# osmosis-diffusion/osmosis-diffusion-code

Measured on AMD Instinct MI355X. Metric: denoise-steps/sec (256x256 RGBD, 1000-step DDPM+guidance), higher is better.
Workload: dtype f32 (f16x3 conv)

## Files before the change

### osmosis_diffusion_code_amd/_lib.py

```python
import ctypes as C
import os
import threading
from typing import List, Optional, Tuple

import torch

_HERE = os.path.dirname(os.path.abspath(__file__))
LIB_PATH = os.environ.get("OSM_LIB") or os.path.join(_HERE, "libosmosis_hip.so")

c_float_p = C.c_void_p


class OsmosisHipError(RuntimeError):
    pass


class ConvDesc(C.Structure):
    _fields_ = [("x", C.c_void_p), ("w", C.c_void_p), ("bias", C.c_void_p), ("res", C.c_void_p),
                ("y", C.c_void_p), ("splitk_ws", C.c_void_p),
                ("B", C.c_int), ("H", C.c_int), ("W", C.c_int), ("Cin", C.c_int), ("Cout", C.c_int),
                ("ksize", C.c_int), ("splitk", C.c_int), ("accumulate", C.c_int),
                ("ldx", C.c_longlong), ("ldy", C.c_longlong), ("ldr", C.c_longlong), ("wfmt", C.c_int),
                ("gn_table", C.c_void_p), ("gn_silu", C.c_int),
                ("colsum", C.c_void_p), ("stat_mode", C.c_int), ("stat_silu", C.c_int), ("stat_x", C.c_void_p),
# ... 153 lines not shown
    "osm_version": [],
}
for _n in ("osm_conv2d_nhwc", "osm_gn_stats", "osm_gn_apply", "osm_gn_fwd", "osm_gn_prep", "osm_gn_bwd", "osm_gn_bwd_apply", "osm_pool2x2",
           "osm_resample_pair", "osm_upsample2x", "osm_stride2_pick", "osm_stride2_place", "osm_add_rowvec", "osm_nchw_to_nhwc", "osm_nhwc_to_nchw", "osm_copy2d"):
    _SIGS[_n + "_h"] = _SIGS[_n]
_SIGS["osm_half_to_f32"] = [_P, _LL, _P, _LL, _LL, _I, _P]
_SIGS["osm_f32_to_half"] = [_P, _LL, _P, _LL, _LL, _I, _P]
EXPORTS = sorted(list(_SIGS) + ["osm_last_error", "osm_packed_weight_elems", "osm_winograd_weight_elems", "osm_quantile_abs_ws_bytes"])
_SIGS_LINOP = {
    "osm_linop_apply": [_P, _P, _P, _P, _P, _P, _I, _I, _LL, _LL, _I, _I, _I, _I, _I, _I, _I, _P],
}
EXPORTS_LINOP = sorted(_SIGS_LINOP)
_SIGS_PSF = {
    "osm_psf_apply": [_P, _P, _P, _P, _P, _I, _I, _I, _I, _I, _LL, _LL, _I, _I, _I, _I, _P],
}
EXPORTS_PSF = sorted(_SIGS_PSF)
_SIGS_PHYSLIN = {
    "osm_phys_forward": [C.POINTER(PhysDesc), _P, _P, _P, _P],
    "osm_phys_resid": [C.POINTER(PhysDesc), _I, _P, _P, _P, _P, _P, _P],
    "osm_phys_reduce_lin": [C.POINTER(PhysDesc), _P, _P, _P, _P, _P],
    "osm_phys_finalize_lin": [C.POINTER(PhysDesc), _I, _P, _P, _P, _P, _I, _P, _P, _I, _P],
    "osm_phys_grad_lin": [C.POINTER(PhysDesc), _I, _P, _P, _P, _P, _P, _I, _P],
    "osm_phys_optimize_lin": [C.POINTER(PhysDesc), C.POINTER(LinDesc), _P, _P, _P, _P, _P, _P, _P, _P, _P, _P, _P, _P, _P, _I, _I, _P, _P],
}
EXPORTS_PHYSLIN = sorted(_SIGS_PHYSLIN)
_SIGS_PHYSGROUP = {
    "osm_phys_finalize_g": [C.POINTER(PhysDesc), C.POINTER(GroupDesc), _P, _P, _P, _I, _P, _P, _I, _P],
    "osm_phys_finalize_lin_g": [C.POINTER(PhysDesc), C.POINTER(GroupDesc), _I, _P, _P, _P, _P, _I, _P, _P, _I, _P],
    "osm_phys_optimize_g": [C.POINTER(PhysDesc), C.POINTER(GroupDesc), _P, _P, _P, _P, _P, _P, _P, _P, _I, _I, _P, _P],
    "osm_phys_optimize_lin_g": [C.POINTER(PhysDesc), C.POINTER(GroupDesc), C.POINTER(LinDesc), _P, _P, _P, _P, _P, _P, _P, _P, _P, _P, _P,
                                _P, _P, _I, _I, _P, _P],
}
EXPORTS_PHYSGROUP = sorted(_SIGS_PHYSGROUP)
_D = C.c_double
_SIGS_BLIND = {
    "osm_psf_tap_grad": [_P, _P, _P, _P, _I, _I, _I, _I, _I, _LL, _LL, _I, _I, _P, _P],
    "osm_psf_tap_step": [_P, _P, _P, _I, _I, _I, _LL, _D, _D, _P],
    "osm_ps_blind_optimize": [_P, _P, _P, _P, _P, _P, _I, _I, _I, _I, _I, _I, _I, _P, _P, _P, _P, _P, _P, _I, _D, _D, _P],
}
EXPORTS_BLIND = sorted(_SIGS_BLIND)
_SIGS_DEPTHPRIOR = {
    "osm_depth_nblk": [_I],
    "osm_depth_reduce": [C.POINTER(DepthDesc), _P, _P, _P, _P, _P],
    "osm_depth_fit": [C.POINTER(DepthDesc), _P, _P, _P, _P],
    "osm_depth_grad": [C.POINTER(DepthDesc), _P, _P, _P, _P, _P, _P],
    "osm_depth_loss_grad": [C.POINTER(DepthDesc), _P, _P, _P, _P, _P, _P, _P, _P],
}
EXPORTS_DEPTHPRIOR = sorted(_SIGS_DEPTHPRIOR)
_SIGS_SOLVER = {
    "osm_solver_update_c": [_P, _P, _P, _P, _P, _P, _P, _P, _P, _F, _P, _P, _P, _I, _I, _I, _P],
    "osm_solver_update_rng_c": [_P, _P, _P, _P, _P, _P, _P, _P, _F, _P, _P, _P, _I, _I, _I, C.c_ulonglong, _P, _I, _I, _I, _I, _P],
}
EXPORTS_SOLVER = sorted(_SIGS_SOLVER)

_lib = None
_lock = threading.Lock()


def load():
    global _lib
    if _lib is not None:
        return _lib
    with _lock:
        if _lib is None:
            if not os.path.exists(LIB_PATH):
                raise OsmosisHipError(
                    f"{LIB_PATH} is missing: build it with `python -c 'import __graft_entry__ as g; g.build()'` "
                    "or `make -C osmosis_diffusion_code_amd/csrc` (hipcc, --offload-arch=gfx950). "
                    "There is no CPU fallback for the product path.")
            lib = C.CDLL(LIB_PATH)
            for name, argtypes in list(_SIGS.items()) + list(_SIGS_LINOP.items()) + list(_SIGS_PSF.items()) + list(_SIGS_PHYSLIN.items()) + \
                    list(_SIGS_PHYSGROUP.items()) + list(_SIGS_BLIND.items()) + list(_SIGS_DEPTHPRIOR.items()) + list(_SIGS_SOLVER.items()):
                fn = getattr(lib, name)
                fn.argtypes = argtypes
                fn.restype = C.c_int
            lib.osm_packed_weight_elems.argtypes = [_I, _I, _I, _I, _I]
            lib.osm_packed_weight_elems.restype = C.c_longlong
            lib.osm_winograd_weight_elems.argtypes = [_I, _I, _I, _I]
            lib.osm_winograd_weight_elems.restype = C.c_longlong
            lib.osm_quantile_abs_ws_bytes.argtypes = [_LL]
            lib.osm_quantile_abs_ws_bytes.restype = C.c_longlong
            lib.osm_last_error.argtypes = []
            lib.osm_last_error.restype = C.c_char_p
            _lib = lib
    return _lib


class Recorder:

    def __init__(self):
        self.calls: List[Tuple] = []
        self.keep: List = []

    def __enter__(self):
        _state.recorders.append(self)
        return self

    def __exit__(self, *exc):
        _state.recorders.pop()
        return False

    @staticmethod
    def suspended():
        class _Suspend:
            def __enter__(self_):
                self_.saved, _state.recorders = _state.recorders, []

            def __exit__(self_, *exc):
                _state.recorders = self_.saved
                return False
        return _Suspend()

    def replay(self):
        for c in self.calls:
            fn, args = c[0], c[1]
            rc = fn(*args)
            if rc != 0:
                raise OsmosisHipError(f"{fn.__name__} failed ({rc}): {load().osm_last_error().decode()}")

    def to_graph(self):
        g = torch.cuda.CUDAGraph()
        cap = torch.cuda.Stream()
        cap.wait_stream(torch.cuda.current_stream())
        with torch.cuda.graph(g, stream=cap):
            cs = torch.cuda.current_stream()
# ... 78 lines not shown
```

### osmosis_diffusion_code_amd/csrc/guidance.hip

```cpp
#include "osm_common.h"
#include "depth_conv.h"
#include "../../include/osmosis_linop.h"
#include "../../include/osmosis_psf.h"
#include "../../include/osmosis_physlin.h"
#include "../../include/osmosis_physgroup.h"
#include "../../include/osmosis_solver.h"

namespace {

constexpr int PPB = 1024;
constexpr int NRED = 16;

template <bool MASKED> struct PixMask { float wm[3]; };
template <> struct PixMask<false> {};

template <bool MASKED>
struct Pix : PixMask<MASKED> {
  float rgb[3], D, y[3];
  float d, dd, w;
  float Ea[3], Eb[3], J[3], r[3];
};

template <bool MASKED, bool FMA_I = false, bool MODEL_ONLY = false>
__device__ __forceinline__ void eval_pixel(const osm_phys_desc& ds, const float* __restrict__ x0,
                                           const float* __restrict__ y, const float* __restrict__ mask,
                                           const float* __restrict__ phi, int b, int p, Pix<MASKED>& q) {
  const long long base = (long long)b * 4 * ds.HW + p;
  float m[3] = {1.f, 1.f, 1.f};
#pragma unroll
  for (int c = 0; c < 3; ++c) {
    q.rgb[c] = x0[base + (long long)c * ds.HW];
    if constexpr (!MODEL_ONLY) q.y[c] = y[(long long)b * 3 * ds.HW + (long long)c * ds.HW + p];
    if constexpr (MASKED) m[c] = mask[(long long)b * 3 * ds.HW + (long long)c * ds.HW + p];
  }
  q.D = x0[base + 3LL * ds.HW];
  if (ds.kind == 3) {
    q.d = 0.f; q.dd = 0.f; q.w = 1.f;
#pragma unroll
    for (int c = 0; c < 3; ++c) {
      q.Ea[c] = q.Eb[c] = 1.f;
      q.J[c] = 0.5f * (q.rgb[c] + 1.0f);
      q.r[c] = q.y[c] - q.rgb[c];
      if constexpr (MASKED) { q.wm[c] = m[c]; q.r[c] *= m[c]; }
    }
    return;
  }
  q.d = conv_depth(q.D, ds.depth_type, ds.dval, q.dd);
  float wdd;
  q.w = ds.weight_type == 1 ? conv_depth(q.D, ds.wdepth_type, ds.wval, wdd) : 1.0f;
  const float* ph = phi + b * 9;
#pragma unroll
  for (int c = 0; c < 3; ++c) {
    const float pa = ds.kind == 2 ? ph[0] : ph[c];
    const float pb = ds.kind == 0 ? ph[3 + c] : pa;
    const float pinf = ph[6 + c];
    q.Ea[c] = expf(-pa * q.d);
    q.Eb[c] = expf(-pb * q.d);
    q.J[c] = 0.5f * (q.rgb[c] + 1.0f);
    float I;
// ... 134 lines not shown
      ph[i] += -lr[i] * (g[i] / (sqrtf(sq) + (float)1e-8));
    }
  } else if (ds.optimizer == 5) {
    for (int i = 0; i < 9; ++i) {
      if (!((live >> i) & 1) || lr[i] == 0.f) continue;
      const float sm = st[i] + g[i] * g[i];
      st[i] = sm;
      ph[i] += -lr[i] * (g[i] / (sqrtf(sm) + (float)1e-10));
    }
  } else if (ds.optimizer == 6) {
    for (int i = 0; i < 9; ++i) {
      if (!((live >> i) & 1) || lr[i] == 0.f) continue;
      const float sq = st[i] * (float)0.9 + (float)(1.0 - 0.9) * g[i] * g[i];
      const float sd = sqrtf(sq + (float)1e-6);
      const float dl = sqrtf(st[9 + i] + (float)1e-6) / sd * g[i];
      st[i] = sq;
      st[9 + i] = st[9 + i] * (float)0.9 + (float)(1.0 - 0.9) * dl * dl;
      ph[i] += -lr[i] * dl;
    }
  } else if (ds.optimizer == 7) {
    const float step = st[19] + 1.f;
    st[19] = step;
    for (int i = 0; i < 9; ++i) {
      if (!((live >> i) & 1) || lr[i] == 0.f) continue;
      const float eta = step == 1.f ? lr[i] : st[i];
      ph[i] *= (float)(1.0 - 1e-4 * (double)eta);
      ph[i] += -eta * g[i];
      st[i] = (float)((double)lr[i] / pow(1.0 + 1e-4 * (double)lr[i] * (double)step, 0.75));
    }
  } else if (ds.optimizer == 8) {
    const float step = st[18] + 1.f;
    st[18] = step;
    for (int i = 0; i < 9; ++i) {
      if (!((live >> i) & 1) || lr[i] == 0.f) continue;
      float ss = step == 1.f ? lr[i] : st[9 + i];
      const float pr = g[i] * st[i];
      float gi = g[i];
      ss *= pr > 0.f ? 1.2f : (pr < 0.f ? 0.5f : 1.f);
      ss = fminf(fmaxf(ss, 1e-6f), 50.f);
      if (pr < 0.f) gi = 0.f;
      ph[i] += -(sgn(gi) * ss);
      st[i] = gi; st[9 + i] = ss;
    }
  } else {
    for (int i = 0; i < 9; ++i)
      if ((live >> i) & 1) ph[i] -= lr[i] * g[i];
  }
  if (ds.kind == 2) ph[1] = ph[2] = ph[0];
}

template <bool LIN> struct FinLin { const float* part_r; int nblk_r, hw; };
template <> struct FinLin<false> {};

template <bool LIN>
__device__ __forceinline__ void fin_walk(const float* __restrict__ part, float* __restrict__ red, int nblk, const FinLin<LIN>& lin,
                                         int b, int lane, double* tot) {
  static_assert(NRED * 4 == 64, "one wave covers the components");
  const int comp = lane >> 2, sub = lane & 3;
  double a = 0.0;
#pragma unroll 4
  for (int k = sub; k < nblk; k += 4) a += (double)part[((long long)b * nblk + k) * NRED + comp];
  if constexpr (LIN) {
    if (comp == 0) {
      a = 0.0;
      for (int k = sub; k < lin.nblk_r; k += 4) a += (double)lin.part_r[(long long)b * lin.nblk_r + k];
    }
  }
  a += __shfl_xor(a, 1, 64);
  a += __shfl_xor(a, 2, 64);
  if (sub == 0) {
    tot[comp] = a;
    red[b * NRED + comp] = (float)a;
  }
}

template <bool LIN>
__device__ __forceinline__ bool fin_member(const osm_phys_desc& ds, const double* tot, const FinLin<LIN>& lin, int zero_guard, int b,
                                           float* __restrict__ loss_out, int do_update, double* dg) {
  double n = 3.0 * (double)ds.HW;
  if constexpr (LIN) n = 3.0 * (double)lin.hw;
  double L, gscale;
  bool live = true;
  if (ds.loss_type == 0) {
    L = sqrt(tot[0]);
    gscale = 1.0 / L;
    if (zero_guard && tot[0] == 0.0) { gscale = 0.0; live = false; }
  } else {
    L = tot[0] / n;
    gscale = 2.0 / n;
  }
  if (loss_out) loss_out[b] = (float)L;
  if (do_update) phys_param_grad(ds, tot, gscale, dg);
  return live;
}

__device__ __forceinline__ void fin_step(const osm_phys_desc& ds, const double* dg, double omega, float* ph, float* st) {
  float g[9], lr[9];
  const int live = phys_param_lr(ds, lr);
  for (int i = 0; i < 9; ++i) g[i] = (float)(dg[i] * omega);
  phys_opt_step(ds, g, lr, live, ph, st);
}

template <bool LIN>
__global__ void phys_finalize_kernel(osm_phys_desc ds, const float* __restrict__ part, float* __restrict__ red,
                                     float* __restrict__ phi, int do_update, float* __restrict__ loss_out,
                                     float* __restrict__ opt_state, int nblk, int zero_guard, const FinLin<LIN> lin) {
  __shared__ double tot[NRED];
  const int b = blockIdx.x;
  fin_walk(part, red, nblk, lin, b, threadIdx.x, tot);
  __syncthreads();
  if (threadIdx.x == 0) {
    double dg[9];
    if (fin_member(ds, tot, lin, zero_guard, b, loss_out, do_update, dg) && do_update)
      fin_step(ds, dg, 1.0, phi + b * 9, opt_state ? opt_state + b * 20 : nullptr);
// ... 56 lines not shown
__global__ __launch_bounds__(256) void phys_grad_kernel(osm_phys_desc ds, const float* __restrict__ x0,
                                                         const float* __restrict__ y,
                                                         const float* __restrict__ mask,
                                                         const float* __restrict__ phi, const float* __restrict__ v,
                                                         const float* __restrict__ red, float* __restrict__ g, int hw,
                                                         int zero_guard) {
  static_assert(!(MASKED && LIN), "the composed route's mask acts on the measurement's grid (phys_resid_kernel)");
  const int b = blockIdx.y;
  const int p = blockIdx.x * 256 + threadIdx.x;
  if (p >= ds.HW) return;
  Pix<MASKED> q;
  eval_pixel<MASKED, MASKED, LIN>(ds, x0, y, mask, phi, b, p, q);
  const float* rd = red + b * NRED;
  const float n = 3.0f * (float)ds.HW;
  float gscale = ds.loss_type == 0 ? 1.0f / sqrtf(rd[0]) : 2.0f / (LIN ? 3.0f * (float)hw : n);
  if ((MASKED || (LIN && zero_guard)) && ds.loss_type == 0 && rd[0] == 0.f) gscale = 0.f;
  const float* ph = phi + b * 9;
  float gD = 0.f;
  const long long base = (long long)b * 4 * ds.HW + p;
  if constexpr (!LIN) {
    if (ds.kind == 3) {
#pragma unroll
      for (int c = 0; c < 3; ++c) {
        if constexpr (MASKED) g[base + (long long)c * ds.HW] = -(q.wm[c] * (q.r[c] * gscale));
        else g[base + (long long)c * ds.HW] = -(q.r[c] * gscale);
      }
      g[base + 3LL * ds.HW] = 0.f;
      return;
    }
  }
#pragma unroll
  for (int c = 0; c < 3; ++c) {
    const float pa = ds.kind == 2 ? ph[0] : ph[c];
    const float pb = ds.kind == 0 ? ph[3 + c] : pa;
    const float pinf = ph[6 + c];
    float dLdI;
    if constexpr (LIN) {
      dLdI = v[((long long)b * 3 + c) * ds.HW + p] * gscale;
    } else {
      float wc = q.w;
      if constexpr (MASKED) wc = q.wm[c];
      dLdI = -2.0f * wc * (q.r[c] * gscale);
    }
    float grgb = dLdI * 0.5f * q.Ea[c];
    if (ds.gamma_avrg != 0.f) grgb += ds.gamma_avrg * sgn(rd[10 + c]) / (float)ds.HW;
    if (ds.gamma_val != 0.f) {
      const float e = fmaxf(fabsf(q.rgb[c]) - 0.7f, 0.0f);
      grgb += ds.gamma_val * 2.0f * e * sgn(q.rgb[c]) / n;
    }
    g[base + (long long)c * ds.HW] = grgb;
    gD += dLdI * (-pa * q.J[c] * q.Ea[c] + pinf * pb * q.Eb[c]) * q.dd;
  }
  g[base + 3LL * ds.HW] = gD;
}


__global__ __launch_bounds__(256) void phys_forward_kernel(osm_phys_desc ds, const float* __restrict__ x0,
                                                            const float* __restrict__ phi, float* __restrict__ F, int P) {
  const int b = blockIdx.y;
  const int p = blockIdx.x * 256 + threadIdx.x;
  if (p >= ds.HW) return;
  Pix<false> q;
  eval_pixel<false, true, true>(ds, x0, nullptr, nullptr, phi, b, p, q);
  const long long base = (long long)b * P * ds.HW + p;
#pragma unroll
  for (int c = 0; c < 3; ++c) F[base + (long long)c * ds.HW] = q.r[c];
  if (P == 4) F[base + 3LL * ds.HW] = q.w;
}

__global__ __launch_bounds__(256) void phys_resid_kernel(const float* __restrict__ AF, const float* __restrict__ y,
                                                          const float* __restrict__ mask, float* __restrict__ u,
                                                          float* __restrict__ part_r, int P, int hw, int nblk) {
  __shared__ float red[4];
  const int b = blockIdx.y, blk = blockIdx.x;
  float s = 0.f;
  const int pend = min(hw, (blk + 1) * PPB);
  for (int p = blk * PPB + threadIdx.x; p < pend; p += 256) {
    const float wt = P == 4 ? AF[((long long)b * P + 3) * hw + p] : 1.0f;
#pragma unroll
    for (int c = 0; c < 3; ++c) {
      const long long e = ((long long)b * 3 + c) * hw + p;
      const float wm = mask ? wt * mask[e] : wt;
      const float r = (y[e] - (2.0f * AF[((long long)b * P + c) * hw + p] - 1.0f)) * wm;
      u[e] = -2.0f * wm * r;
      s += r * r;
    }
  }
  const float t = osm::wave_sum(s);
  if ((threadIdx.x & 63) == 0) red[threadIdx.x >> 6] = t;
  __syncthreads();
  if (threadIdx.x == 0) part_r[(long long)b * nblk + blk] = (red[0] + red[1]) + (red[2] + red[3]);
}

template <int MK, int VK, bool RAW>
__global__ __launch_bounds__(256) void posterior_kernel(const float* __restrict__ mo, const float* __restrict__ x,
                                                           const float* __restrict__ coef, float* __restrict__ x0_raw,
                                                           float* __restrict__ x0, float* __restrict__ mean,
                                                           float* __restrict__ logvar, int B, int C, int Cout, int HW) {
  const long long n = (long long)C * HW, no = (long long)Cout * HW;
  const long long total = (long long)B * n;
  const long long voff = Cout == C ? 0 : n;
  const float c0 = coef[0], c1 = coef[1], c2 = coef[2], c3 = coef[3], mn = coef[4], mxl = coef[5];
  for (long long i = (long long)blockIdx.x * blockDim.x + threadIdx.x; i < total;
       i += (long long)gridDim.x * blockDim.x) {
    const long long b = i / n;
    const long long rem = i - b * n;
// ... 561 lines not shown
  return phys_grad_launch("osm_phys_grad_lin", d, x0, nullptr, nullptr, phi, red, g, stream, &la, masked != 0);
}

namespace {
struct LinWs { const osm_lin_desc* lin; float *F, *AF, *u, *v, *part_r; };

int phys_optimize_launch(const char* who, const osm_phys_desc* d, const float* x0, const float* y, const float* mask, float* phi,
                         float* part, float* red, float* loss_out, float* g, int n_inner, int freeze_phi, float* opt_state,
                         void* stream, const GroupOff* go = nullptr, const LinWs* lw = nullptr) {
  int rc = lw ? check_lin_desc(d, who) : check_desc(d, who);
  if (rc) return rc;
  if (lw && (rc = check_lin(d, lw->lin, who))) return rc;
  OSM_REQUIRE(x0 && y && phi && part && red && loss_out && g && (!lw || (lw->F && lw->AF && lw->u && lw->v && lw->part_r)),
              "%s: null pointer", who);
  OSM_REQUIRE(n_inner >= 1, "%s: n_inner must be >= 1", who);
  OSM_REQUIRE(!(freeze_phi && n_inner != 1), "%s: freeze_phi goes with n_inner = 1", who);
  if ((rc = check_phi_step(who, d, !freeze_phi, opt_state))) return rc;
  OSM_REQUIRE(!lw || (long long)d->B * 4 <= 65535, "%s: batch %d is too large for one launch of the operator", who, d->B);
  const int zg = mask != nullptr, hw = lw ? lw->lin->h * lw->lin->w : 0, P = lin_planes(d);
  const LinArgs la_{hw, lw ? lw->v : nullptr, lw ? lw->part_r : nullptr}, *la = lw ? &la_ : nullptr;
  for (int it = 0; it < n_inner; ++it) {
    if (lw) {
      if ((rc = osm_phys_forward(d, x0, phi, lw->F, stream))) return rc;
      if ((rc = lin_apply(lw->lin, lw->F, lw->AF, d->B, P, 0, stream))) return rc;
      if ((rc = osm_phys_resid(d, hw, lw->AF, y, mask, lw->u, lw->part_r, stream))) return rc;
      if ((rc = lin_apply(lw->lin, lw->u, lw->v, d->B, 3, 1, stream))) return rc;
    }
    if ((rc = phys_reduce_launch(who, d, x0, y, mask, phi, part, stream, la))) return rc;
    if (it < n_inner - 1) {
      if ((rc = phys_finalize_launch(who, d, part, red, phi, 1, loss_out, opt_state, zg, stream, go, la))) return rc;
      continue;
    }
    if ((rc = phys_finalize_launch(who, d, part, red, phi, 0, loss_out, nullptr, zg, stream, go, la))) return rc;
    if ((rc = phys_grad_launch(who, d, x0, y, mask, phi, red, g, stream, la, zg))) return rc;
    if (!freeze_phi && (rc = phys_finalize_launch(who, d, part, red, phi, 1, nullptr, opt_state, zg, stream, go, la))) return rc;
  }
  return OSM_OK;
}
}

extern "C" int osm_phys_optimize(const osm_phys_desc* d, const float* x0, const float* y, float* phi, float* part, float* red,
                                 float* loss_out, float* g, int n_inner, int freeze_phi, float* opt_state, void* stream) {
  return phys_optimize_launch("osm_phys_optimize", d, x0, y, nullptr, phi, part, red, loss_out, g, n_inner, freeze_phi, opt_state,
                              stream);
}

extern "C" int osm_phys_optimize_m(const osm_phys_desc* d, const float* x0, const float* y, const float* mask, float* phi, float* part,
                                   float* red, float* loss_out, float* g, int n_inner, int freeze_phi, float* opt_state,
                                   void* stream) {
  return phys_optimize_launch("osm_phys_optimize_m", d, x0, y, mask, phi, part, red, loss_out, g, n_inner, freeze_phi, opt_state,
                              stream);
}

extern "C" int osm_phys_optimize_lin(const osm_phys_desc* d, const osm_lin_desc* lin, const float* x0, const float* y, const float* mask,
                                     float* phi, float* F, float* AF, float* u, float* v, float* part_r, float* part, float* red,
                                     float* loss_out, float* g, int n_inner, int freeze_phi, float* opt_state, void* stream) {
  const LinWs lw{lin, F, AF, u, v, part_r};
  return phys_optimize_launch("osm_phys_optimize_lin", d, x0, y, mask, phi, part, red, loss_out, g, n_inner, freeze_phi, opt_state,
                              stream, nullptr, &lw);
}

extern "C" int osm_phys_finalize_g(const osm_phys_desc* d, const osm_group_desc* grp, const float* part, float* red, float* phi,
                                   int do_update, float* loss_out, float* opt_state, int masked, void* stream) {
  const char* who = "osm_phys_finalize_g";
  GroupOff go;
  int rc = check_desc(d, who);
  if (rc) return rc;
  if ((rc = check_group(d, grp, &go, who))) return rc;
  return phys_finalize_launch(who, d, part, red, phi, do_update, loss_out, opt_state, masked != 0, stream, &go);
}

extern "C" int osm_phys_finalize_lin_g(const osm_phys_desc* d, const osm_group_desc* grp, int hw, const float* part, const float* part_r,
                                       float* red, float* phi, int do_update, float* loss_out, float* opt_state, int masked,
                                       void* stream) {
  const char* who = "osm_phys_finalize_lin_g";
  GroupOff go;
  int rc = check_lin_desc(d, who);
  if (rc) return rc;
  if ((rc = check_group(d, grp, &go, who))) return rc;
  const LinArgs la{hw, nullptr, part_r};
  return phys_finalize_launch(who, d, part, red, phi, do_update, loss_out, opt_state, masked != 0, stream, &go, &la);
}

extern "C" int osm_phys_optimize_g(const osm_phys_desc* d, const osm_group_desc* grp, const float* x0, const float* y, const float* mask,
                                   float* phi, float* part, float* red, float* loss_out, float* g, int n_inner, int freeze_phi,
                                   float* opt_state, void* stream) {
  const char* who = "osm_phys_optimize_g";
  GroupOff go;
  int rc = check_desc(d, who);
  if (rc) return rc;
  if ((rc = check_group(d, grp, &go, who))) return rc;
  return phys_optimize_launch(who, d, x0, y, mask, phi, part, red, loss_out, g, n_inner, freeze_phi, opt_state, stream, &go);
}

extern "C" int osm_phys_optimize_lin_g(const osm_phys_desc* d, const osm_group_desc* grp, const osm_lin_desc* lin, const float* x0,
                                       const float* y, const float* mask, float* phi, float* F, float* AF, float* u, float* v,
                                       float* part_r, float* part, float* red, float* loss_out, float* g, int n_inner, int freeze_phi,
                                       float* opt_state, void* stream) {
  const char* who = "osm_phys_optimize_lin_g";
  GroupOff go;
  int rc = check_lin_desc(d, who);
  if (rc) return rc;
  if ((rc = check_group(d, grp, &go, who))) return rc;
  const LinWs lw{lin, F, AF, u, v, part_r};
  return phys_optimize_launch(who, d, x0, y, mask, phi, part, red, loss_out, g, n_inner, freeze_phi, opt_state, stream, &go, &lw);
}
// ... 439 lines not shown
```

### osmosis_diffusion_code_amd/guided_diffusion/condition_methods.py

```python
from abc import ABC, abstractmethod
from functools import partial

import os
import torch

from .. import ops
from .._lib import PhysDesc
from ..osmosis_utils import losses as losseso
from ..osmosis_utils import utils as utilso

__CONDITIONING_METHOD__ = {}


def register_conditioning_method(name: str):
    def wrapper(cls):
        if __CONDITIONING_METHOD__.get(name, None):
            raise NameError(f"Name {name} is already registered!")
        __CONDITIONING_METHOD__[name] = cls
        return cls
    return wrapper


def get_conditioning_method(name: str, operator, noiser, **kwargs):
    if __CONDITIONING_METHOD__.get(name, None) is None:
# ... 314 lines not shown
            return None
        B, _, H, W = x_0_hat.shape
        z, m = self.depth_prior_rows(B, H, W, x_0_hat.device)
        L, reported, a, c = depth_prior_term(self._depth_torch(x_0_hat[:, 3:4]), z.view(B, 1, H, W).to(x_0_hat.dtype),
                                             m.view(B, 1, H, W).to(x_0_hat.dtype), dp["align"], dp["loss"], dp["scale"], dp["scale_min"])
        with torch.no_grad():
            dp["out_loss"].copy_(reported)
            dp["out_fit"][:, 0].copy_(a)
            dp["out_fit"][:, 1].copy_(c)
        return dp["weight"] * L.sum()

    def _degradation(self):
        from .measurements import GRID_OPERATORS
        deg = getattr(self.operator, "degradation", None)
        return deg if isinstance(deg, GRID_OPERATORS) else None

    def _prepare(self, B, HW, device, grid=None):
        key = (B, HW, str(device)) if grid is None else (B, HW, str(device), int(grid[0]), int(grid[1]))
        st = self._states.get(key)
        if st is not None:
            self._state = st
            return st
        op = self.operator
        if not hasattr(op, "fill_desc"):
            raise NotImplementedError(f"operator {type(op).__name__} has no HIP physics kernels")
        if self.loss_function not in ("norm", "mse"):
            raise NotImplementedError
        d = PhysDesc()
        op.fill_desc(d)
        if self.loss_weight in (None, "none"):
            d.weight_type, d.wdepth_type = 0, 0
        elif self.loss_weight == "depth":
            fn, value = utilso.parse_weight_function(self.weight_function)
            code, vals = utilso.depth_code_and_values(fn if fn != "none" else None, value)
            d.weight_type, d.wdepth_type = 1, code
            for i in range(3):
                d.wval[i] = vals[i]
        else:
            raise NotImplementedError
        d.loss_type = 0 if self.loss_function == "norm" else 1
        coefs = self.aux_loss.kernel_coefficients() if self.aux_loss is not None else {"gamma_avrg": 0.0, "gamma_val": 0.0}
        d.gamma_avrg, d.gamma_val = coefs["gamma_avrg"], coefs["gamma_val"]
        d.B, d.HW = B, HW
        from .measurements import OPTIMIZER_CODES
        d.optimizer = OPTIMIZER_CODES.get(getattr(op, "optimizer", "") or "", 0)
        nblk = ops.phys_nblk(HW)
        if d.optimizer != 0 and (self._opt is None or self._opt.shape[0] != op.phi.shape[0] or self._opt.device != op.phi.device):
            self._opt = torch.zeros(op.phi.shape[0], 20, device=device, dtype=torch.float32)
        st = {"key": key, "desc": d,
              "part": torch.empty(B * nblk * 16, device=device, dtype=torch.float32),
              "red": torch.zeros(B * 16, device=device, dtype=torch.float32),
              "loss": torch.zeros(B, device=device, dtype=torch.float32),
              "g": torch.empty(B, 4, HW, device=device, dtype=torch.float32)}
        if grid is not None:
            lin = ops.lin_desc(self._degradation(), grid[0], grid[1], device)
            hw, P = lin.h * lin.w, ops.phys_lin_planes(d)
            f32 = dict(device=device, dtype=torch.float32)
            st.update(lin=lin, hw=hw, F=torch.empty(B, P, HW, **f32), AF=torch.empty(B, P, hw, **f32), u=torch.empty(B, 3, hw, **f32),
                      v=torch.empty(B, 3, HW, **f32), part_r=torch.empty(B * ops.phys_nblk(hw), **f32))
        while len(self._states) >= 4:
            self._states.pop(next(iter(self._states)))
        self._states[st["key"]] = st
        self._state = st
        return st

    def _group(self, phi):
        sizes = getattr(self.operator, "group_sizes", None)
        if sizes is None:
            return None
        full = self.operator.phi
        if phi.data_ptr() != full.data_ptr() or phi.shape[0] != full.shape[0]:
            raise ValueError(f"phi_groups: a water group spans chunks -- the data term got {phi.shape[0]} phi rows of the operator's "
                             f"{full.shape[0]}; a grouped batch takes ONE call over all its images")
        key = (sizes, self.operator.phi_reduce)
        if getattr(self, "_grp_key", None) != key:
            self._grp, self._grp_key = ops.group_desc(sizes, self.operator.phi_reduce), key
        return self._grp

    def loss_grad_x0(self, x0, y, freeze_phi=False, g_out=None, phi=None, loss_out=None, mask=None, depth=None):
        if getattr(self.operator, "degradation", None) is not None:
            return self._loss_grad_x0_lin(x0, y, freeze_phi, g_out, phi, loss_out, mask, depth)
        B, HW = x0.shape[0], x0.shape[2] * x0.shape[3]
        if y.shape[0] != B or y.shape[1] != 3 or x0.shape[1] != 4:
            raise ValueError("expected x0 [B,4,H,W] and measurement [B,3,H,W]")
        grp = self._group(self.operator.phi if phi is None else phi)
        depth = self._depth_rows(x0, depth) if (self._depth is not None or depth is not None) else None
        st = self._prepare(B, HW, x0.device)
        d, part, red, loss = st["desc"], st["part"], st["red"], st["loss"]
        opt = self._opt if d.optimizer != 0 else None
        if loss_out is not None:
            loss = loss_out
        phi = self.operator.phi if phi is None else phi
        if phi.shape[0] != B or not phi.is_contiguous():
            raise ValueError("phi must be a contiguous [B][9] block")
        g = g_out if g_out is not None else st["g"]
        x0c, yc = x0.contiguous(), y.contiguous()
        if mask is None:
            mask = self.measurement_mask(B, HW, x0.device)
        if grp is not None:
            route = (partial(ops.phys_reduce_m, d, x0c, yc, mask, phi, part),
                     partial(ops.phys_finalize_g, d, grp, part, red, phi, masked=mask is not None),
                     partial(ops.phys_grad_m, d, x0c, yc, mask, phi, red, g),
                     partial(ops.phys_optimize_g, d, grp, x0c, yc, mask, phi, part, red, loss, g))
        elif mask is not None:
            route = (partial(ops.phys_reduce_m, d, x0c, yc, mask, phi, part), partial(ops.phys_finalize_m, d, part, red, phi),
                     partial(ops.phys_grad_m, d, x0c, yc, mask, phi, red, g),
                     partial(ops.phys_optimize_m, d, x0c, yc, mask, phi, part, red, loss, g))
        else:
            route = (partial(ops.phys_reduce, d, x0c, yc, phi, part), partial(ops.phys_finalize, d, part, red, phi),
                     partial(ops.phys_grad, d, x0c, yc, phi, red, g),
                     partial(ops.phys_optimize, d, x0c, yc, phi, part, red, loss, g))
        self._inner_loop(route, 1 if freeze_phi else self.n_iter, freeze_phi, loss, self._opt_rows(opt, phi))
        if depth is not None:
            self._apply_depth_prior(st, x0c, g, depth)
        return g.view(x0.shape), loss

    @staticmethod
    def _inner_loop(route, n_inner, freeze_phi, loss, rows):
        reduce, finalize, grad, optimize = route
        if os.environ.get("OSM_PHYS_PY_LOOP", "0") != "1":
            optimize(n_inner, freeze_phi, opt_state=rows)
            return
        for it in range(n_inner):
            reduce()
            if it < n_inner - 1:
                finalize(True, loss, opt_state=rows)
                continue
            finalize(False, loss)
            grad()
            if not freeze_phi:
                finalize(True, None, opt_state=rows)

    def _loss_grad_x0_lin(self, x0, y, freeze_phi=False, g_out=None, phi=None, loss_out=None, mask=None, depth=None):
        deg = self._degradation()
        if deg is None:
            raise NotImplementedError(f"degradation {type(self.operator.degradation).__name__} has no HIP kernels (autograd conditioning "
                                      "serves it)")
        if x0.dim() != 4 or x0.shape[1] != 4:
            raise ValueError(f"expected x0 [B,4,H,W], got {tuple(x0.shape)}")
        B, _, H, W = x0.shape
        h, w = deg.out_shape(H, W)
        if tuple(y.shape) != (B, 3, h, w):
            raise ValueError(f"expected the measurement [{B},3,{h},{w}] (the degradation's grid for a {H} x {W} image), got {tuple(y.shape)}")
        HW, hw = H * W, h * w
        grp = self._group(self.operator.phi if phi is None else phi)
        depth = self._depth_rows(x0, depth) if (self._depth is not None or depth is not None) else None
        st = self._prepare(B, HW, x0.device, grid=(H, W))
        d, lin, part, red, loss = st["desc"], st["lin"], st["part"], st["red"], st["loss"]
        F, AF, u, v, part_r = st["F"], st["AF"], st["u"], st["v"], st["part_r"]
        opt = self._opt if d.optimizer != 0 else None
        if loss_out is not None:
            loss = loss_out
        phi = self.operator.phi if phi is None else phi
        if phi.shape[0] != B or not phi.is_contiguous():
            raise ValueError("phi must be a contiguous [B][9] block")
        g = g_out if g_out is not None else st["g"]
        x0c, yc = x0.contiguous(), y.contiguous()
        if mask is None:
            if self._mask is not None and self._mask.shape[2] != hw:
                raise ValueError(f"measurement mask [{self._mask.shape[0]},3,{self._mask.shape[2]}] does not fit a measurement "
                                 f"[{B},3,{h},{w}] (the mask lives on the measurement's grid)")
            mask = self.measurement_mask(B, hw, x0.device)
        elif mask.numel() != B * 3 * hw:
            raise ValueError(f"expected mask rows [{B},3,{hw}] (the measurement's grid {h} x {w}), got {tuple(mask.shape)}")
        P, masked = ops.phys_lin_planes(d), mask is not None
# ... 302 lines not shown
```

### osmosis_diffusion_code_amd/ops.py

```python
import ctypes as C
from dataclasses import dataclass
from typing import Optional

import torch

from . import _lib
from ._lib import AttnDesc, ConvDesc, DepthDesc, GemmDesc, GroupDesc, LinDesc, PhysDesc, ReconDesc, call, current_stream_ptr, ptr, ptr_f64, query


@dataclass
class Mat:
    t: torch.Tensor
    rows: int
    cols: int
    ld: int

    @staticmethod
    def of(t: torch.Tensor) -> "Mat":
        if t.dim() != 2 or (t.shape[1] > 1 and t.stride(1) != 1):
            raise _lib.OsmosisHipError("Mat.of needs a 2-D view with unit column stride")
        return Mat(t, t.shape[0], t.shape[1], t.stride(0) if t.shape[0] > 1 else max(t.stride(0), t.shape[1]))

    @property
    def p(self) -> int:
# ... 343 lines not shown
    assert g.numel() == x_raw.numel() and g.is_contiguous() and x_raw.is_contiguous()
    call("osm_dynthr_bwd", ptr(g), ptr(x_raw), ptr(q), ptr(idx), float(s), g.numel(), ptr(ws), _s(), keep=(g, x_raw, q, idx, ws))


def phys_nblk(HW):
    return query("osm_phys_nblk", HW)


def phys_reduce(desc: PhysDesc, x0, y, phi, part):
    call("osm_phys_reduce", C.byref(desc), ptr(x0), ptr(y), ptr(phi), ptr(part), _s(), keep=(desc, x0, y, phi, part))


def phys_finalize(desc: PhysDesc, part, red, phi, do_update, loss_out, opt_state=None):
    call("osm_phys_finalize", C.byref(desc), ptr(part), ptr(red), ptr(phi), int(do_update), ptr(loss_out), ptr(opt_state), _s(),
         keep=(part, red, phi, loss_out, opt_state))


def phys_grad(desc: PhysDesc, x0, y, phi, red, g):
    call("osm_phys_grad", C.byref(desc), ptr(x0), ptr(y), ptr(phi), ptr(red), ptr(g), _s(),
         keep=(desc, x0, y, phi, red, g))


def phys_optimize(desc: PhysDesc, x0, y, phi, part, red, loss_out, g, n_inner: int, freeze_phi: bool, opt_state=None):
    call("osm_phys_optimize", C.byref(desc), ptr(x0), ptr(y), ptr(phi), ptr(part), ptr(red), ptr(loss_out), ptr(g), int(n_inner),
         int(bool(freeze_phi)), ptr(opt_state), _s(), keep=(desc, x0, y, phi, part, red, loss_out, g, opt_state))


def _check_mask(mask, y):
    if mask is not None and (mask.numel() != y.numel() or not mask.is_contiguous() or mask.dtype != torch.float32):
        raise ValueError(f"mask must be contiguous fp32 with the measurement's {y.numel()} elements ([B,3,HW]), "
                         f"got {tuple(mask.shape)} {mask.dtype}")


def phys_reduce_m(desc: PhysDesc, x0, y, mask, phi, part):
    _check_mask(mask, y)
    call("osm_phys_reduce_m", C.byref(desc), ptr(x0), ptr(y), ptr(mask), ptr(phi), ptr(part), _s(), keep=(desc, x0, y, mask, phi, part))


def phys_finalize_m(desc: PhysDesc, part, red, phi, do_update, loss_out, opt_state=None, masked=True):
    call("osm_phys_finalize_m", C.byref(desc), ptr(part), ptr(red), ptr(phi), int(do_update), ptr(loss_out), ptr(opt_state),
         int(bool(masked)), _s(), keep=(part, red, phi, loss_out, opt_state))


def phys_grad_m(desc: PhysDesc, x0, y, mask, phi, red, g):
    _check_mask(mask, y)
    call("osm_phys_grad_m", C.byref(desc), ptr(x0), ptr(y), ptr(mask), ptr(phi), ptr(red), ptr(g), _s(),
         keep=(desc, x0, y, mask, phi, red, g))


def phys_optimize_m(desc: PhysDesc, x0, y, mask, phi, part, red, loss_out, g, n_inner: int, freeze_phi: bool, opt_state=None):
    _check_mask(mask, y)
    call("osm_phys_optimize_m", C.byref(desc), ptr(x0), ptr(y), ptr(mask), ptr(phi), ptr(part), ptr(red), ptr(loss_out), ptr(g),
         int(n_inner), int(bool(freeze_phi)), ptr(opt_state), _s(), keep=(desc, x0, y, mask, phi, part, red, loss_out, g, opt_state))


def exposure_mask(y, mask_out, B, HW, low, high, soft=0.0, per_pixel=False):
    assert y.numel() == B * 3 * HW and mask_out.numel() == B * 3 * HW and y.is_contiguous() and mask_out.is_contiguous()
    call("osm_exposure_mask", ptr(y), float(low), float(high), float(soft), int(bool(per_pixel)), ptr(mask_out), B, HW, _s(),
         keep=(y, mask_out))


def posterior_bwd(g, coef, d_out, B, HW):
    call("osm_posterior_bwd", ptr(g), ptr(coef), ptr(d_out), B, HW, _s(), keep=(g, coef, d_out))


def guide_update(mean, logvar, g, dx_unet, noise, coef, scale4, clip, x_next, grad_out, B, HW):
    call("osm_guide_update", ptr(mean), ptr(logvar), ptr(g), ptr(dx_unet), ptr(noise), ptr(coef), ptr(scale4),
         float(clip), ptr(x_next), ptr(grad_out), B, HW, _s(),
         keep=(mean, logvar, g, dx_unet, noise, coef, scale4, x_next, grad_out))


def guide_update_rng(mean, logvar, g, dx_unet, coef, scale4, clip, x_next, grad_out, noise_out, B, HW, seed, step, step_offset=0,
                     img0=0, img_stride=1):
    call("osm_guide_update_rng", ptr(mean), ptr(logvar), ptr(g), ptr(dx_unet), ptr(coef), ptr(scale4), float(clip), ptr(x_next),
         ptr(grad_out), ptr(noise_out), B, HW, int(seed) & 0xFFFFFFFFFFFFFFFF, ptr(step), int(step_offset), int(img0), int(img_stride), _s(),
         keep=(mean, logvar, g, dx_unet, coef, scale4, x_next, grad_out, noise_out, step))


def guide_update_rng_sub(mean, logvar, g, dx_unet, coef, scale4, clip, x_next, grad_out, noise_out, B, HW, seed, step, step_offset=0,
                         sub=0, img0=0, img_stride=1):
    call("osm_guide_update_rng_sub", ptr(mean), ptr(logvar), ptr(g), ptr(dx_unet), ptr(coef), ptr(scale4), float(clip), ptr(x_next),
         ptr(grad_out), ptr(noise_out), B, HW, int(seed) & 0xFFFFFFFFFFFFFFFF, ptr(step), int(step_offset), int(sub), int(img0),
         int(img_stride), _s(), keep=(mean, logvar, g, dx_unet, coef, scale4, x_next, grad_out, noise_out, step))


def randn(out, B, n, seed, step=None, step_const=0, img0=0, img_stride=1):
    call("osm_randn", ptr(out), int(B), int(n), int(seed) & 0xFFFFFFFFFFFFFFFF, ptr(step), int(step_const), int(img0), int(img_stride), _s(),
         keep=(out, step))


def randn_sub(out, B, n, seed, step=None, step_const=0, sub=0, img0=0, img_stride=1):
    call("osm_randn_sub", ptr(out), int(B), int(n), int(seed) & 0xFFFFFFFFFFFFFFFF, ptr(step), int(step_const), int(sub), int(img0),
         int(img_stride), _s(), keep=(out, step))


def philox_raw(out, n4, c1, c2, c3, k0, k1):
    call("osm_philox_raw", ptr(out), int(n4), int(c1), int(c2), int(c3), int(k0), int(k1), _s(), keep=(out,))


def ddim_update(x0, x, g, dx_unet, noise, coef, dcoef, scale4, clip, x_next, grad_out, B, HW):
    call("osm_ddim_update", ptr(x0), ptr(x), ptr(g), ptr(dx_unet), ptr(noise), ptr(coef), ptr(dcoef), ptr(scale4), float(clip),
         ptr(x_next), ptr(grad_out), B, HW, _s(), keep=(x0, x, g, dx_unet, noise, coef, dcoef, scale4, x_next, grad_out))


def fetch_coefs(table, step, delta, coef_out, t_out, B):
    call("osm_fetch_coefs", ptr(table), int(table.shape[0]), ptr(step), delta, ptr(coef_out), ptr(t_out), B, _s(),
# ... 409 lines not shown
```

Baseline: 54.22.

## Add persistent resident kernel for physics phi inner optimization loop

Adds a persistent kernel that keeps each block's pixel data in registers across all inner iterations of the phi optimization. Blocks exchange per-iteration partial sums through a global workspace with atomic counters and a spin-wait, and every block finalizes phi redundantly, so the per-iteration reduce/finalize kernel launches are replaced by one launch. The goal is to remove launch overhead and the repeated global reloads of x0, y and mask. It depends on all blocks being co-resident (checked against occupancy), and it adds a timeout abort that writes NaN, plus a new workspace buffer.

```diff
diff --git a/include/osmosis_physresident.h b/include/osmosis_physresident.h
--- /dev/null
+++ b/include/osmosis_physresident.h
@@ -0,0 +1,18 @@
+#ifndef OSMOSIS_PHYSRESIDENT_H
+#define OSMOSIS_PHYSRESIDENT_H
+
+#include "osmosis_hip.h"
+
+#ifdef __cplusplus
+extern "C" {
+#endif
+
+int osm_phys_resident_ws_bytes(int B, int HW);
+int osm_phys_resident_supported(const osm_phys_desc* d, int n_inner, int masked);
+int osm_phys_optimize_r(const osm_phys_desc* d, const float* x0, const float* y, const float* mask , float* phi, float* part,
+                        float* red, float* loss_out, float* g, int n_inner, int freeze_phi, float* opt_state, void* ws, void* stream);
+
+#ifdef __cplusplus
+}
+#endif
+#endif
diff --git a/osmosis_diffusion_code_amd/_lib.py b/osmosis_diffusion_code_amd/_lib.py
--- a/osmosis_diffusion_code_amd/_lib.py
+++ b/osmosis_diffusion_code_amd/_lib.py
@@ -229,6 +229,12 @@
     "osm_solver_update_rng_c": [_P, _P, _P, _P, _P, _P, _P, _P, _F, _P, _P, _P, _I, _I, _I, C.c_ulonglong, _P, _I, _I, _I, _I, _P],
 }
 EXPORTS_SOLVER = sorted(_SIGS_SOLVER)
+_SIGS_PHYSRESIDENT = {
+    "osm_phys_resident_ws_bytes": [_I, _I],
+    "osm_phys_resident_supported": [C.POINTER(PhysDesc), _I, _I],
+    "osm_phys_optimize_r": [C.POINTER(PhysDesc), _P, _P, _P, _P, _P, _P, _P, _P, _I, _I, _P, _P, _P],
+}
+EXPORTS_PHYSRESIDENT = sorted(_SIGS_PHYSRESIDENT)
 
 _lib = None
 _lock = threading.Lock()
@@ -247,7 +253,8 @@
                     "There is no CPU fallback for the product path.")
             lib = C.CDLL(LIB_PATH)
             for name, argtypes in list(_SIGS.items()) + list(_SIGS_LINOP.items()) + list(_SIGS_PSF.items()) + list(_SIGS_PHYSLIN.items()) + \
-                    list(_SIGS_PHYSGROUP.items()) + list(_SIGS_BLIND.items()) + list(_SIGS_DEPTHPRIOR.items()) + list(_SIGS_SOLVER.items()):
+                    list(_SIGS_PHYSGROUP.items()) + list(_SIGS_BLIND.items()) + list(_SIGS_DEPTHPRIOR.items()) + list(_SIGS_SOLVER.items()) + \
+                    list(_SIGS_PHYSRESIDENT.items()):
                 fn = getattr(lib, name)
                 fn.argtypes = argtypes
                 fn.restype = C.c_int
diff --git a/osmosis_diffusion_code_amd/csrc/guidance.hip b/osmosis_diffusion_code_amd/csrc/guidance.hip
--- a/osmosis_diffusion_code_amd/csrc/guidance.hip
+++ b/osmosis_diffusion_code_amd/csrc/guidance.hip
@@ -5,6 +5,7 @@
 #include "../../include/osmosis_physlin.h"
 #include "../../include/osmosis_physgroup.h"
 #include "../../include/osmosis_solver.h"
+#include "../../include/osmosis_physresident.h"
 
 namespace {
 
@@ -245,14 +246,31 @@
 template <bool LIN> struct FinLin { const float* part_r; int nblk_r, hw; };
 template <> struct FinLin<false> {};
 
-template <bool LIN>
+__device__ __forceinline__ float load_sc1(const float* p) {
+  return __builtin_bit_cast(float, __hip_atomic_load(reinterpret_cast<unsigned*>(const_cast<float*>(p)), __ATOMIC_RELAXED,
+                                                     __HIP_MEMORY_SCOPE_AGENT));
+}
+
+template <bool LIN, bool SC1 = false>
 __device__ __forceinline__ void fin_walk(const float* __restrict__ part, float* __restrict__ red, int nblk, const FinLin<LIN>& lin,
                                          int b, int lane, double* tot) {
   static_assert(NRED * 4 == 64, "one wave covers the components");
   const int comp = lane >> 2, sub = lane & 3;
   double a = 0.0;
+  if constexpr (SC1) {
+    for (int k0 = sub; k0 < nblk; k0 += 64) {
+      float v[16];
+#pragma unroll
+      for (int j = 0; j < 16; ++j)
+        if (k0 + 4 * j < nblk) v[j] = load_sc1(part + ((long long)b * nblk + k0 + 4 * j) * NRED + comp);
+#pragma unroll
+      for (int j = 0; j < 16; ++j)
+        if (k0 + 4 * j < nblk) a += (double)v[j];
+    }
+  } else {
 #pragma unroll 4
-  for (int k = sub; k < nblk; k += 4) a += (double)part[((long long)b * nblk + k) * NRED + comp];
+    for (int k = sub; k < nblk; k += 4) a += (double)part[((long long)b * nblk + k) * NRED + comp];
+  }
   if constexpr (LIN) {
     if (comp == 0) {
       a = 0.0;
@@ -415,6 +433,224 @@
     gD += dLdI * (-pa * q.J[c] * q.Ea[c] + pinf * pb * q.Eb[c]) * q.dd;
   }
   g[base + 3LL * ds.HW] = gD;
+}
+
+constexpr int RPT = PPB / 256;
+constexpr int RES_HDR = 16;
+constexpr int RES_CNT = 32;
+constexpr long long RES_WAIT_TICKS = 2000000;
+
+__host__ __device__ inline long long res_phi_off(int B) { return RES_HDR + (long long)RES_CNT * B; }
+__host__ __device__ inline long long res_slot_off(int B) { return res_phi_off(B) + ((long long)B * 9 + 15) / 16 * 16; }
+__host__ __device__ inline long long res_rowp_off(int B, int nblk) { return res_slot_off(B) + 2LL * B * nblk * NRED; }
+__host__ __device__ inline long long res_rows_off(int B, int nblk) { return res_rowp_off(B, nblk) + ((long long)B * nblk * 9 + 15) / 16 * 16; }
+__host__ __device__ inline long long res_ws_words(int B, int nblk) {
+  return res_rows_off(B, nblk) + ((long long)B * nblk * 20 + 15) / 16 * 16;
+}
+
+typedef unsigned res_u32x4 __attribute__((ext_vector_type(4)));
+
+template <bool MASKED>
+__device__ __forceinline__ void res_pixel_terms(int kind, const float* ph, float d, float w, const float* wm, const float* J,
+                                                const float* y, float* s) {
+#pragma clang fp contract(off)
+  float r[3], k2[3], Ea[3], Eb[3];
+#pragma unroll
+  for (int c = 0; c < 3; ++c) {
+    const float pa = kind == 2 ? ph[0] : ph[c];
+    const float pb = kind == 0 ? ph[3 + c] : pa;
+    Ea[c] = expf(-pa * d);
+    Eb[c] = expf(-pb * d);
+    const float tb = ph[6 + c] * (1.0f - Eb[c]);
+    const float I = c < 2 ? fmaf(J[c], Ea[c], tb) : J[c] * Ea[c] + tb;
+    const float wc = MASKED ? wm[c] : w;
+    r[c] = (y[c] - (2.0f * I - 1.0f)) * wc;
+    k2[c] = -2.0f * wc * r[c];
+  }
+  s[0] = fmaf(r[0], r[0], s[0]);
+  s[0] = fmaf(r[1], r[1], s[0]);
+  s[0] = s[0] + r[2] * r[2];
+#pragma unroll
+  for (int c = 0; c < 3; ++c) {
+    const float da = -d * J[c] * Ea[c];
+    const float db = ph[6 + c] * d * Eb[c];
+    s[1 + c] = c == 0 ? s[1] + k2[0] * da : fmaf(k2[c], da, s[1 + c]);
+    s[4 + c] = fmaf(k2[c], db, s[4 + c]);
+    s[7 + c] = fmaf(k2[c], 1.0f - Eb[c], s[7 + c]);
+  }
+}
+
+__device__ __forceinline__ void res_pixel_fixed(const float* rgb, float* s) {
+#pragma clang fp contract(off)
+#pragma unroll
+  for (int c = 0; c < 3; ++c) {
+    s[10 + c] = s[10 + c] + rgb[c];
+    const float e = fmaxf(fabsf(rgb[c]) - 0.7f, 0.0f);
+    s[13] = c == 0 ? fmaf(e, e, s[13]) : s[13] + e * e;
+  }
+}
+
+__device__ __forceinline__ int res_wait(unsigned* cnt, unsigned target, unsigned* abort_w) {
+  const long long t0 = wall_clock64();
+  for (;;) {
+    const unsigned c = __hip_atomic_load(cnt, __ATOMIC_RELAXED, __HIP_MEMORY_SCOPE_AGENT);
+    if (__hip_atomic_load(abort_w, __ATOMIC_RELAXED, __HIP_MEMORY_SCOPE_AGENT) != 0u) return 0;
+    if (c >= target) return 1;
+    if (wall_clock64() - t0 > RES_WAIT_TICKS) {
+      __hip_atomic_store(abort_w, 1u, __ATOMIC_RELAXED, __HIP_MEMORY_SCOPE_AGENT);
+      return 0;
+    }
+    __builtin_amdgcn_s_sleep(1);
+  }
+}
+
+__device__ __noinline__ void res_finalize_lane(const osm_phys_desc ds, const double* __restrict__ tot, int zero_guard,
+                                               float* __restrict__ loss_out, int do_update, float* __restrict__ phi,
+                                               float* __restrict__ opt_state) {
+  double dg[9];
+  if (fin_member(ds, tot, FinLin<false>{}, zero_guard, 0, loss_out, do_update, dg) && do_update)
+    fin_step(ds, dg, 1.0, phi, opt_state);
+}
+
+template <bool MASKED>
+__global__ __launch_bounds__(256) void phys_resident_kernel(osm_phys_desc ds, const float* __restrict__ x0,
+                                                             const float* __restrict__ y, const float* __restrict__ mask,
+                                                             float* phi, float* red, float* loss_out, float* opt_state, int n_inner,
+                                                             int freeze_phi, unsigned* ws, int nblk) {
+  __shared__ float red_sh[4][NRED];
+  __shared__ double tot[NRED];
+  __shared__ float redf[NRED], row_ph[9], loss_sh;
+  __shared__ int ok_sh;
+  const int b = blockIdx.y, blk = blockIdx.x, tid = threadIdx.x, lane = tid & 63, wv = tid >> 6;
+  unsigned* abort_w = ws;
+  unsigned* cnt = ws + RES_HDR + RES_CNT * b;
+  float* phi_last = reinterpret_cast<float*>(ws + res_phi_off(ds.B)) + b * 9;
+  const long long slot_off = res_slot_off(ds.B);
+  const __amdgpu_buffer_rsrc_t rsrc = __builtin_amdgcn_make_buffer_rsrc(ws, 0, 0x7fffffff, 0x00020000);
+  float* my_ph = reinterpret_cast<float*>(ws + res_rowp_off(ds.B, nblk)) + ((long long)b * nblk + blk) * 9;
+  float* my_st = reinterpret_cast<float*>(ws + res_rows_off(ds.B, nblk)) + ((long long)b * nblk + blk) * 20;
+
+  if (tid < 9) row_ph[tid] = my_ph[tid] = phi[b * 9 + tid];
+  if (opt_state && tid < 20) my_st[tid] = opt_state[b * 20 + tid];
+  if (tid == 0) ok_sh = __hip_atomic_load(abort_w, __ATOMIC_RELAXED, __HIP_MEMORY_SCOPE_AGENT) == 0u;
+
+  const int pend = min(ds.HW, (blk + 1) * PPB), p0 = blk * PPB + tid;
+  float pd[RPT], pw[RPT], pJ[RPT][3], py[RPT][3], pwm[RPT][3];
+  float s[NRED];
+#pragma unroll
+  for (int k = 0; k < NRED; ++k) s[k] = 0.f;
+#pragma unroll
+  for (int i = 0; i < RPT; ++i) {
+    const int p = p0 + 256 * i;
+    pd[i] = 0.f; pw[i] = 0.f;
+#pragma unroll
+    for (int c = 0; c < 3; ++c) { pJ[i][c] = 0.f; py[i][c] = 0.f; pwm[i][c] = 0.f; }
+    if (p < pend) {
+      const long long base = (long long)b * 4 * ds.HW + p;
+      float rgb[3], m[3] = {1.f, 1.f, 1.f};
+#pragma unroll
+      for (int c = 0; c < 3; ++c) {
+        rgb[c] = x0[base + (long long)c * ds.HW];
+        py[i][c] = y[(long long)b * 3 * ds.HW + (long long)c * ds.HW + p];
+        if constexpr (MASKED) m[c] = mask[(long long)b * 3 * ds.HW + (long long)c * ds.HW + p];
+      }
+      const float D = x0[base + 3LL * ds.HW];
+      float dd, wdd;
+      pd[i] = conv_depth(D, ds.depth_type, ds.dval, dd);
+      pw[i] = ds.weight_type == 1 ? conv_depth(D, ds.wdepth_type, ds.wval, wdd) : 1.0f;
+#pragma unroll
+      for (int c = 0; c < 3; ++c) {
+        pJ[i][c] = 0.5f * (rgb[c] + 1.0f);
+        if constexpr (MASKED) pwm[i][c] = pw[i] * m[c];
+      }
+      res_pixel_fixed(rgb, s);
+    }
+  }
+#pragma unroll
+  for (int k = 10; k < NRED; ++k) {
+    const float t = osm::wave_sum(s[k]);
+    if (lane == 0) red_sh[wv][k] = t;
+  }
+  __syncthreads();
+
+  bool ok = ok_sh != 0;
+  for (int it = 0; ok && it < n_inner; ++it) {
+    float ph[9];
+#pragma unroll
+    for (int i = 0; i < 9; ++i) ph[i] = row_ph[i];
+#pragma unroll
+    for (int k = 0; k < 10; ++k) s[k] = 0.f;
+#pragma unroll
+    for (int i = 0; i < RPT; ++i)
+      if (p0 + 256 * i < pend) res_pixel_terms<MASKED>(ds.kind, ph, pd[i], pw[i], pwm[i], pJ[i], py[i], s);
+#pragma unroll
+    for (int k = 0; k < 10; ++k) {
+      const float t = osm::wave_sum(s[k]);
+      if (lane == 0) red_sh[wv][k] = t;
+    }
+    __syncthreads();
+    if (wv == 0) {
+      const long long img = slot_off + ((long long)(it & 1) * ds.B + b) * nblk * NRED;
+      if (lane < 4) {
+        float v[4];
+#pragma unroll
+        for (int j = 0; j < 4; ++j) {
+          const int k = 4 * lane + j;
+          v[j] = (red_sh[0][k] + red_sh[1][k]) + (red_sh[2][k] + red_sh[3][k]);
+        }
+        const res_u32x4 bits = {__builtin_bit_cast(unsigned, v[0]), __builtin_bit_cast(unsigned, v[1]),
+                                __builtin_bit_cast(unsigned, v[2]), __builtin_bit_cast(unsigned, v[3])};
+        __builtin_amdgcn_raw_buffer_store_b128(bits, rsrc, (int)((img + (long long)blk * NRED + 4 * lane) * 4), 0, 16);
+      }
+      asm volatile("s_waitcnt vmcnt(0)" ::: "memory");
+      int here = 1;
+      if (nblk > 1) {
+        if (lane == 0) {
+          __hip_atomic_fetch_add(cnt, 1u, __ATOMIC_RELAXED, __HIP_MEMORY_SCOPE_AGENT);
+          here = res_wait(cnt, (unsigned)(it + 1) * (unsigned)nblk, abort_w);
+        }
+        here = __shfl(here, 0, 64);
+      }
+      __builtin_amdgcn_fence(__ATOMIC_ACQUIRE, "wavefront");
+      if (here) {
+        fin_walk<false, true>(reinterpret_cast<const float*>(ws) + img, redf, nblk, FinLin<false>{}, 0, lane, tot);
+        __builtin_amdgcn_wave_barrier();
+        if (lane == 0) {
+          const bool last = it == n_inner - 1;
+          const int do_update = last ? !freeze_phi : 1;
+          if (last && blk == 0)
+            for (int i = 0; i < 9; ++i) phi_last[i] = row_ph[i];
+          res_finalize_lane(ds, tot, MASKED ? 1 : 0, &loss_sh, do_update, my_ph, opt_state ? my_st : nullptr);
+          for (int i = 0; i < 9; ++i) row_ph[i] = my_ph[i];
+        }
+      }
+      if (lane == 0) ok_sh = here;
+    }
+    __syncthreads();
+    ok = ok_sh != 0;
+  }
+
+  if (!ok) {
+    const float nan = __builtin_nanf("");
+    if (tid == 0) loss_out[b] = nan;
+    if (tid < 9) phi_last[tid] = nan;
+    if (tid < NRED) red[b * NRED + tid] = nan;
+    return;
+  }
+  if (blk == 0) {
+    if (tid < NRED) red[b * NRED + tid] = redf[tid];
+    if (tid == 0) loss_out[b] = loss_sh;
+    if (!freeze_phi) {
+      if (tid < 9) phi[b * 9 + tid] = row_ph[tid];
+      if (opt_state && tid < 20) opt_state[b * 20 + tid] = my_st[tid];
+    }
+  }
+  if (nblk > 1 && tid == 0) {
+    if (__hip_atomic_fetch_add(cnt + 1, 1u, __ATOMIC_RELAXED, __HIP_MEMORY_SCOPE_AGENT) == (unsigned)nblk - 1u) {
+      __hip_atomic_store(cnt, 0u, __ATOMIC_RELAXED, __HIP_MEMORY_SCOPE_AGENT);
+      __hip_atomic_store(cnt + 1, 0u, __ATOMIC_RELAXED, __HIP_MEMORY_SCOPE_AGENT);
+    }
+  }
 }
 
 
@@ -1082,6 +1318,67 @@
                               stream);
 }
 
+namespace {
+int res_admits(bool masked) {
+  static int cap[2] = {-1, -1};
+  int& c = cap[masked ? 1 : 0];
+  if (c >= 0) return c;
+  int dev = 0, cus = 0, occ = 0;
+  hipError_t e = hipGetDevice(&dev);
+  if (e == hipSuccess) e = hipDeviceGetAttribute(&cus, hipDeviceAttributeMultiprocessorCount, dev);
+  if (e == hipSuccess) {
+    e = masked ? hipOccupancyMaxActiveBlocksPerMultiprocessor(&occ, phys_resident_kernel<true>, 256, 0)
+               : hipOccupancyMaxActiveBlocksPerMultiprocessor(&occ, phys_resident_kernel<false>, 256, 0);
+  }
+  if (e != hipSuccess) {
+    (void)hipGetLastError();
+    return 0;
+  }
+  const long long half = (long long)occ * cus / 2;
+  c = (int)(half < cus ? half : cus);
+  return c;
+}
+}
+
+extern "C" int osm_phys_resident_ws_bytes(int B, int HW) {
+  if (B < 1 || HW < 1) return -1;
+  const long long bytes = res_ws_words(B, osm_phys_nblk(HW)) * 4;
+  return bytes > 0x7fffffffLL ? -1 : (int)bytes;
+}
+
+extern "C" int osm_phys_resident_supported(const osm_phys_desc* d, int n_inner, int masked) {
+  if (!d || d->kind < 0 || d->kind > 2 || d->B < 1 || d->HW < 1 || n_inner < 1) return 0;
+  if (osm_phys_resident_ws_bytes(d->B, d->HW) < 0) return 0;
+  return (long long)d->B * osm_phys_nblk(d->HW) <= res_admits(masked != 0) ? 1 : 0;
+}
+
+extern "C" int osm_phys_optimize_r(const osm_phys_desc* d, const float* x0, const float* y, const float* mask, float* phi, float* part,
+                                   float* red, float* loss_out, float* g, int n_inner, int freeze_phi, float* opt_state, void* ws,
+                                   void* stream) {
+  const char* who = "osm_phys_optimize_r";
+  int rc = check_desc(d, who);
+  if (rc) return rc;
+  OSM_REQUIRE(x0 && y && phi && part && red && loss_out && g && ws, "%s: null pointer", who);
+  OSM_REQUIRE(n_inner >= 1, "%s: n_inner must be >= 1", who);
+  OSM_REQUIRE(!(freeze_phi && n_inner != 1), "%s: freeze_phi goes with n_inner = 1", who);
+  if ((rc = check_phi_step(who, d, !freeze_phi, opt_state))) return rc;
+  if (!osm_phys_resident_supported(d, n_inner, mask != nullptr))
+    return phys_optimize_launch(who, d, x0, y, mask, phi, part, red, loss_out, g, n_inner, freeze_phi, opt_state, stream);
+  const int nblk = osm_phys_nblk(d->HW);
+  const dim3 grid(nblk, d->B), block(256);
+  hipStream_t st = (hipStream_t)stream;
+  if (mask) {
+    hipLaunchKernelGGL(phys_resident_kernel<true>, grid, block, 0, st, *d, x0, y, mask, phi, red, loss_out, opt_state, n_inner,
+                       freeze_phi, (unsigned*)ws, nblk);
+  } else {
+    hipLaunchKernelGGL(phys_resident_kernel<false>, grid, block, 0, st, *d, x0, y, nullptr, phi, red, loss_out, opt_state, n_inner,
+                       freeze_phi, (unsigned*)ws, nblk);
+  }
+  if ((rc = osm::check_launch("phys_resident_kernel"))) return rc;
+  const float* phi_last = reinterpret_cast<const float*>(ws) + res_phi_off(d->B);
+  return phys_grad_launch(who, d, x0, y, mask, phi_last, red, g, stream, nullptr, mask != nullptr);
+}
+
 extern "C" int osm_phys_optimize_lin(const osm_phys_desc* d, const osm_lin_desc* lin, const float* x0, const float* y, const float* mask,
                                      float* phi, float* F, float* AF, float* u, float* v, float* part_r, float* part, float* red,
                                      float* loss_out, float* g, int n_inner, int freeze_phi, float* opt_state, void* stream) {
diff --git a/osmosis_diffusion_code_amd/guided_diffusion/condition_methods.py b/osmosis_diffusion_code_amd/guided_diffusion/condition_methods.py
--- a/osmosis_diffusion_code_amd/guided_diffusion/condition_methods.py
+++ b/osmosis_diffusion_code_amd/guided_diffusion/condition_methods.py
@@ -390,6 +390,8 @@
               "red": torch.zeros(B * 16, device=device, dtype=torch.float32),
               "loss": torch.zeros(B, device=device, dtype=torch.float32),
               "g": torch.empty(B, 4, HW, device=device, dtype=torch.float32)}
+        if grid is None:
+            st["ws"] = torch.zeros((ops.phys_resident_ws_bytes(B, HW) + 3) // 4, device=device, dtype=torch.int32)
         if grid is not None:
             lin = ops.lin_desc(self._degradation(), grid[0], grid[1], device)
             hw, P = lin.h * lin.w, ops.phys_lin_planes(d)
@@ -448,7 +450,10 @@
             route = (partial(ops.phys_reduce, d, x0c, yc, phi, part), partial(ops.phys_finalize, d, part, red, phi),
                      partial(ops.phys_grad, d, x0c, yc, phi, red, g),
                      partial(ops.phys_optimize, d, x0c, yc, phi, part, red, loss, g))
-        self._inner_loop(route, 1 if freeze_phi else self.n_iter, freeze_phi, loss, self._opt_rows(opt, phi))
+        n_inner = 1 if freeze_phi else self.n_iter
+        if grp is None and os.environ.get("OSM_PHI_RESIDENT", "1") != "0" and ops.phys_resident_supported(d, n_inner, mask is not None):
+            route = route[:3] + (partial(ops.phys_optimize_r, d, x0c, yc, mask, phi, part, red, loss, g, ws=st["ws"]),)
+        self._inner_loop(route, n_inner, freeze_phi, loss, self._opt_rows(opt, phi))
         if depth is not None:
             self._apply_depth_prior(st, x0c, g, depth)
         return g.view(x0.shape), loss
diff --git a/osmosis_diffusion_code_amd/ops.py b/osmosis_diffusion_code_amd/ops.py
--- a/osmosis_diffusion_code_amd/ops.py
+++ b/osmosis_diffusion_code_amd/ops.py
@@ -419,6 +419,23 @@
     _check_mask(mask, y)
     call("osm_phys_optimize_m", C.byref(desc), ptr(x0), ptr(y), ptr(mask), ptr(phi), ptr(part), ptr(red), ptr(loss_out), ptr(g),
          int(n_inner), int(bool(freeze_phi)), ptr(opt_state), _s(), keep=(desc, x0, y, mask, phi, part, red, loss_out, g, opt_state))
+
+
+def phys_resident_ws_bytes(B, HW):
+    return query("osm_phys_resident_ws_bytes", int(B), int(HW))
+
+
+def phys_resident_supported(desc: PhysDesc, n_inner: int, masked: bool):
+    return bool(query("osm_phys_resident_supported", C.byref(desc), int(n_inner), int(bool(masked))))
+
+
+def phys_optimize_r(desc: PhysDesc, x0, y, mask, phi, part, red, loss_out, g, n_inner: int, freeze_phi: bool, opt_state=None, ws=None):
+    _check_mask(mask, y)
+    if ws is None or ws.dtype != torch.int32 or ws.numel() * 4 < phys_resident_ws_bytes(desc.B, desc.HW):
+        raise ValueError("phys_optimize_r: ws must be an int32 tensor of phys_resident_ws_bytes(B, HW) bytes")
+    call("osm_phys_optimize_r", C.byref(desc), ptr(x0), ptr(y), ptr(mask), ptr(phi), ptr(part), ptr(red), ptr(loss_out), ptr(g),
+         int(n_inner), int(bool(freeze_phi)), ptr(opt_state), ptr(ws), _s(),
+         keep=(desc, x0, y, mask, phi, part, red, loss_out, g, opt_state, ws))
 
 
 def exposure_mask(y, mask_out, B, HW, low, high, soft=0.0, per_pixel=False):
```

Result: no change. 54.44 (median of 6 runs) (+0.4%).
